# JuliaLinearAlgebra/ArnoldiMethod.jl

Measured on AMD Instinct MI355X. Metric: arnoldi_iters_per_sec, higher is better.
Workload: dtype f64

## Files before the change

### arnoldimethod.jl_amd/build.py

```python
from __future__ import annotations

import os
import shutil
import subprocess
from concurrent.futures import ThreadPoolExecutor

HERE = os.path.dirname(os.path.abspath(__file__))
CSRC = os.path.join(HERE, "csrc")
SRC = os.path.join(CSRC, "ks_hip.hip")
BLK = os.path.join(CSRC, "ks_block_inst.hip")
HEADERS = [os.path.join(CSRC, f) for f in ("ks_kernels.hpp", "ks_spmv_march.hpp", "ks_p2p.hpp", "ks_driver.hpp", "ks_smalldense.hpp", "ks_context.hpp", "ks_host_defs.hpp", "ks_csr_layout.hpp", "ks_halo_plan.hpp", "ks_halo.hpp", "ks_operators.hpp", "ks_sptrsv.hpp", "ks_tridiag_plan.hpp", "ks_tridiag.hpp", "ks_product.hpp", "ks_grid.hpp", "ks_grid_var.hpp", "ks_grid_box.hpp",
                                           "ks_workspace.hpp", "ks_backend.hpp", "ks_vectors.hpp", "ks_block.hpp", "ks_block_kernels.hpp", "ks_block_launch.hpp", "ks_block_mfma.hpp")]
DEPS = [SRC, BLK] + HEADERS + [os.path.join(HERE, "..", "include", "kschur.h")]
OUT = os.path.join(HERE, "libkschur_hip.so")
OBJDIR = os.path.join(HERE, "build")
BLK_DEPS = [BLK] + [os.path.join(CSRC, f) for f in ("ks_kernels.hpp", "ks_host_defs.hpp", "ks_p2p.hpp", "ks_block_kernels.hpp", "ks_block_launch.hpp", "ks_block_mfma.hpp")]
UNITS = {
    "ks_hip.o": (SRC, [], DEPS),
    "ks_block_inst0.o": (BLK, ["-DKS_BLK_PART=0"], BLK_DEPS),
    "ks_block_inst1.o": (BLK, ["-DKS_BLK_PART=1"], BLK_DEPS),
    "ks_block_inst2.o": (BLK, ["-DKS_BLK_PART=2"], BLK_DEPS),
}


def hipcc() -> str:
    for cand in (shutil.which("hipcc"), "/opt/rocm/bin/hipcc"):
        if cand and os.path.exists(cand):
            return cand
    raise RuntimeError("hipcc not found")


def needs_build() -> bool:
    if not os.path.exists(OUT):
        return True
    t = os.path.getmtime(OUT)
    return any(os.path.getmtime(d) > t for d in DEPS)


def _stale(obj: str, deps) -> bool:
    if not os.path.exists(obj):
        return True
    t = os.path.getmtime(obj)
    return any(os.path.getmtime(d) > t for d in deps)


def build(force: bool = False, verbose: bool = False) -> str:
    if not force and not needs_build():
        return OUT
    os.makedirs(OBJDIR, exist_ok=True)
    cc = hipcc()
    extra = os.environ.get("KS_EXTRA_HIPCC_FLAGS", "").split()
    jobs = []
    for name, (src, flags, deps) in UNITS.items():
        obj = os.path.join(OBJDIR, name)
        if force or extra or _stale(obj, deps):
            jobs.append([cc, "--offload-arch=gfx950", "-O3", "-std=c++17", "-fPIC", "-c", src, "-o", obj] + flags + extra)

    def run(cmd):
        if verbose:
            print(" ".join(cmd), flush=True)
        subprocess.check_call(cmd, cwd=CSRC)

    with ThreadPoolExecutor(max_workers=max(1, min(len(jobs), os.cpu_count() or 1))) as ex:
        list(ex.map(run, jobs))
    link = [cc, "--offload-arch=gfx950", "-shared", "-fPIC"] + [os.path.join(OBJDIR, n) for n in UNITS] + ["-o", OUT, "-L/opt/rocm/lib", "-lrccl", "-Wl,-rpath,/opt/rocm/lib"]
    run(link)
    return OUT


if __name__ == "__main__":
    print(build(force=True, verbose=True))
```

### arnoldimethod.jl_amd/csrc/ks_hip.hip

```cpp
#include <hip/hip_runtime.h>
#include <rccl/rccl.h>

#include <signal.h>
#include <unistd.h>

#include <algorithm>
#include <chrono>
#include <cmath>
#include <cstdio>
#include <cstdlib>
#include <cstring>
#include <memory>
#include <stdexcept>
#include <string>
#include <thread>
#include <unordered_map>
#include <vector>

#include "../../include/kschur.h"
#include "ks_driver.hpp"
#include "ks_kernels.hpp"
#include "ks_spmv_march.hpp"
#include "ks_block_kernels.hpp"
#include "ks_block_launch.hpp"

using ks::cplx;
using ksd::cd;
using ksd::DevState;
using ksd::kBlock;

#include "ks_context.hpp"
#include "ks_csr_layout.hpp"
#include "ks_halo_plan.hpp"
#include "ks_halo.hpp"
#include "ks_operators.hpp"
#include "ks_sptrsv.hpp"
#include "ks_tridiag.hpp"
#include "ks_product.hpp"
#include "ks_grid.hpp"
#include "ks_grid_var.hpp"
#include "ks_grid_box.hpp"
#include "ks_workspace.hpp"
#include "ks_block.hpp"
#include "ks_backend.hpp"
#include "ks_vectors.hpp"

namespace {

template <class F> int grid_operator_entry(ks_ctx* ctx, int dtype, ks_operator** out, const std::string& who, F make) {
  return guarded([&] {
    KS_REQUIRE(ctx && out, KS_ERR_ARGUMENT, "null argument");
    KS_REQUIRE(dtype == KS_F64 || dtype == KS_C64, KS_ERR_ARGUMENT, "unknown dtype");
    KS_REQUIRE(!ctx->distributed() && ctx->nranks == 1, KS_ERR_ARGUMENT, who + ": single-GPU contexts only (the grid is not partitioned across ranks)");
    ctx->use();
    *out = dtype == KS_F64 ? make(double{}, who) : make(cd{}, who);
  });
}

template <class F> int grid_host_entry(int dtype, const std::string& who, F fill) {
  return guarded([&] {
    KS_REQUIRE(dtype == KS_F64 || dtype == KS_C64, KS_ERR_ARGUMENT, "unknown dtype");
    if (dtype == KS_F64) fill(double{}, who);
    else fill(cplx{}, who);
  });
}

}

extern "C" {

const char* ks_last_error_string(void) { return g_last_error.c_str(); }

int ks_version(int* major, int* minor) {
  if (major) *major = KS_VERSION_MAJOR;
  if (minor) *minor = KS_VERSION_MINOR;
  return KS_OK;
}

int ks_ctx_create(int device, ks_ctx** out) {
  return guarded([&] {
    KS_REQUIRE(out, KS_ERR_ARGUMENT, "null out");
    auto c = std::make_unique<ks_ctx>();
    ctx_init_device(c.get(), device);
    *out = c.release();
  });
}

int ks_comm_unique_id(void* out128) {
  return guarded([&] {
    static_assert(sizeof(ncclUniqueId) == 128, "ncclUniqueId is 128 bytes");
    ncclUniqueId id;
    KS_NCCL(ncclGetUniqueId(&id));
    std::memcpy(out128, &id, 128);
  });
}

int ks_ctx_create_dist(int device, int rank, int nranks, const void* unique_id128, ks_ctx** out) {
  return guarded([&] {
    KS_REQUIRE(out && unique_id128, KS_ERR_ARGUMENT, "null argument");
    KS_REQUIRE(nranks >= 1 && rank >= 0 && rank < nranks, KS_ERR_ARGUMENT, "bad rank/nranks");
    auto c = std::make_unique<ks_ctx>();
    ctx_init_device(c.get(), device);
    c->rank = rank;
    c->nranks = nranks;
    ncclUniqueId id;
    std::memcpy(&id, unique_id128, 128);
    KS_NCCL(ncclCommInitRank(&c->comm, nranks, id, rank));
    const char* tr = std::getenv("KS_TRANSPORT");
    if (tr && std::string(tr) == "p2p") {
      p2p_alloc(c.get());
      hipIpcMemHandle_t mine;
      KS_HIP(hipIpcGetMemHandle(&mine, c->p2p.region));
      char* dbuf = nullptr;
      KS_HIP(hipMalloc(&dbuf, (size_t)64 * nranks));
      KS_HIP(hipMemcpy(dbuf + (size_t)64 * rank, &mine, 64, hipMemcpyHostToDevice));
      KS_NCCL(ncclAllGather(dbuf + (size_t)64 * rank, dbuf, 64, ncclChar, c->comm, c->stream));
      std::vector<char> all((size_t)64 * nranks);
      KS_HIP(hipMemcpyAsync(all.data(), dbuf, all.size(), hipMemcpyDeviceToHost, c->stream));
      KS_HIP(hipStreamSynchronize(c->stream));
      (void)hipFree(dbuf);
      p2p_attach(c.get(), all.data());
    }
    *out = c.release();
  });
}

int ks_ctx_create_hostcomm(int device, int rank, int nranks, ks_host_allreduce_fn allreduce, ks_host_exchange_fn exchange,
                           void* user, ks_ctx** out) {
  return guarded([&] {
    KS_REQUIRE(out && allreduce && exchange, KS_ERR_ARGUMENT, "null argument");
    KS_REQUIRE(nranks >= 1 && rank >= 0 && rank < nranks, KS_ERR_ARGUMENT, "bad rank/nranks");
    auto c = std::make_unique<ks_ctx>();
    ctx_init_device(c.get(), device);
    c->rank = rank;
    c->nranks = nranks;
    c->hc.allreduce = allreduce;
    c->hc.exchange = exchange;
    c->hc.user = user;
    *out = c.release();
  });
}

int ks_ctx_create_p2p(int device, int rank, int nranks, ks_ctx** out) {
  return guarded([&] {
    KS_REQUIRE(out, KS_ERR_ARGUMENT, "null out");
    KS_REQUIRE(nranks >= 1 && rank >= 0 && rank < nranks, KS_ERR_ARGUMENT, "bad rank/nranks");
    auto c = std::make_unique<ks_ctx>();
    ctx_init_device(c.get(), device);
    c->rank = rank;
    c->nranks = nranks;
    p2p_alloc(c.get());
    if (nranks == 1) p2p_attach(c.get(), nullptr);
    *out = c.release();
  });
}

int ks_ctx_p2p_handle(ks_ctx* ctx, void* out64) {
  return guarded([&] {
    KS_REQUIRE(ctx && out64, KS_ERR_ARGUMENT, "null argument");
    KS_REQUIRE(ctx->p2p.allocated, KS_ERR_ARGUMENT, "context was not created with ks_ctx_create_p2p");
    ctx->use();
    hipIpcMemHandle_t h;
    KS_HIP(hipIpcGetMemHandle(&h, ctx->p2p.region));
    std::memcpy(out64, &h, 64);
  });
}

int ks_ctx_p2p_attach(ks_ctx* ctx, const void* handles) {
  return guarded([&] {
    KS_REQUIRE(ctx && handles, KS_ERR_ARGUMENT, "null argument");
    ctx->use();
    p2p_attach(ctx, handles);
  });
}

int ks_ctx_destroy(ks_ctx* ctx) {
  return guarded([&] {
    if (!ctx) return;
    (void)hipSetDevice(ctx->device);
    if (ctx->stream) (void)hipStreamSynchronize(ctx->stream);
    if (ctx->comm) (void)ncclCommDestroy(ctx->comm);
    if (ctx->hc.stage) (void)hipHostFree(ctx->hc.stage);
    if (ctx->operr_h) (void)hipHostFree(ctx->operr_h);
    p2p_release(ctx);
    if (ctx->stream) (void)hipStreamDestroy(ctx->stream);
    delete ctx;
// ... 1579 lines not shown
```

### arnoldimethod.jl_amd/csrc/ks_operators.hpp

```cpp
#pragma once
struct ks_operator {
  ks_ctx* ctx = nullptr;
  int64_t n_local = 0, nnz = 0;
  int dtype = KS_F64;
  bool async_capable = true;
  double bytes_per_nnz = 0.0;
  double aux_bytes = 0.0;
  int layout = -1;
  double in_scale = 1.0;
  bool shift_store_cacheable = false;
  virtual ~ks_operator() = default;
  virtual void apply(const void* x, void* y, const DevState* st) = 0;
  virtual void apply_shifted(const void* x, void* y, double theta_re, double theta_im, double sigma, int64_t ld, const DevState* st);
};

namespace {

template <class D> struct CsrOp : ks_operator {
  void* rowptr = nullptr;
  bool ptr64 = false;
  int32_t* colidx = nullptr;
  D* val = nullptr;
  void* blkptr = nullptr;
  int32_t* blkrow = nullptr;
  int nblk = 0;
  std::vector<std::unique_ptr<CsrOp<D>>> cblocks;
  std::vector<char> cb_from_ghost;
  int cb_rpt = 0, cb_ni = 0;
  int ni = 7;
  bool row_gather = false;
  int nlong = 0;
  int32_t* blkpart = nullptr;
  D* lpart = nullptr;
  int32_t* lrow = nullptr;
  int32_t* lfirst = nullptr;
  int nstencil = 0;
  int stencil_mask_bytes = 1;
  void* smask = nullptr;
  void* smask2 = nullptr;
  ksd::StencilDict<D> sdict{};
  int nstencil_local = 0;
  mutable bool split_said = false;
  void* sliceptr = nullptr;
  int32_t* sperm = nullptr;
  int nslices = 0;
  int sell_un = 8;
  int64_t sell_entries = 0;
  int ndict = 0;
  int ndvi = 0;
  uint8_t* codes = nullptr;
  int32_t* ddelta = nullptr;
  int dvi_unroll = 8;
  int dvi_rpt = 1;
  Halo<D> halo;

  ~CsrOp() override {
    (void)hipFree(rowptr); (void)hipFree(colidx); (void)hipFree(val); (void)hipFree(blkptr); (void)hipFree(blkrow); (void)hipFree(smask); (void)hipFree(sliceptr); (void)hipFree(sperm); (void)hipFree(blkpart); (void)hipFree(lpart); (void)hipFree(lrow); (void)hipFree(lfirst);
    (void)hipFree(codes); (void)hipFree(ddelta);
  }
  void launch_csr_blocks(const D* x, D* y, const DevState* st, const D* yacc, int plain_store, ksd::ShiftArg<D> shift = ksd::ShiftArg<D>{}) {
    hipStream_t s = ctx->stream;
    auto go = [&](auto ip_tag) {
      using IP = decltype(ip_tag);
      auto launch = [&](auto ni_tag) {
        constexpr int NI = decltype(ni_tag)::value;
        if constexpr ((size_t)NI * kBlock * sizeof(D) <= (size_t)ksd::kSpmvCapBytes)
          ksd::k_spmv_csr<D, IP, false, NI><<<nblk, kBlock, 0, s>>>(static_cast<const IP*>(blkptr), blkrow, static_cast<const IP*>(rowptr), colidx, val, x,
                                                                    nullptr, y, n_local, nblk, st, nullptr, 0, 0, nullptr, nullptr, yacc, plain_store,
                                                                    ksd::HaloFused{}, ksd::HaloArgs{}, ksd::P2pDev{}, env_int("KS_SPMV_CSR_NT", 1) != 0, row_gather,
                                                                    plain_store ? ksd::ShiftArg<D>{} : shift);
        else
          throw KsError{KS_ERR_INTERNAL, "CSR row blocks of " + std::to_string(NI) + " x 256 entries exceed the LDS budget of this element type"};
      };
      switch (ni) {
        case 4: launch(std::integral_constant<int, 4>{}); break;
        case 7: launch(std::integral_constant<int, 7>{}); break;
        case 8: launch(std::integral_constant<int, 8>{}); break;
        case 12: launch(std::integral_constant<int, 12>{}); break;
        default: launch(std::integral_constant<int, 16>{}); break;
      }
    };
    if (ptr64) go(int64_t{});
    else go(int32_t{});
  }
  bool shift_on = false;
  D shift_theta{};
  double shift_sigma = 1.0;
  bool shift_plain() const {
    static const int env = env_int("KS_SHIFT_PLAIN", -1);
    return env >= 0 ? env != 0 : shift_store_cacheable;
  }
  static bool march_on() {
    return env_int("KS_STENCIL_MARCH", 1) != 0;
  }
  int march_slots(int ntiles) const {
    const int env = env_int("KS_MARCH_S", 0);
    int S = 192;
    if (env > 0) S = env;
    else {
      int64_t P = 0;
      for (int k = 0; k < nstencil; ++k) P = std::max<int64_t>(P, std::llabs((long long)sdict.delta[k]));
      const int64_t per = P / 512 + 1;
      if (per >= 16 && per <= 224) S = (int)(per * ((160 + per - 1) / per)) <= 224 ? (int)(per * ((160 + per - 1) / per)) : (int)per;
    }
    S = std::min(S, std::max(1, (ntiles + 7) / 8));
    return S;
  }
  void launch_march(const D* x, D* y, int nt, const DevState* st, hipStream_t s) const {
    if constexpr (std::is_same<D, double>::value) {
      const int sh = shift_on ? (1 | (shift_plain() ? 2 : 0)) : 0;
      const uint16_t* m2 = static_cast<const uint16_t*>(smask2);
      const int G = 8 * march_slots(nt);
      int kown = -1;
      for (int k = 0; k < nstencil; ++k)
        if (sdict.delta[k] == 0) kown = k;
      auto go = [&](auto ns_tag, auto ko_tag) {
        ksd::k_spmv_stencil_march<decltype(ns_tag)::value, decltype(ko_tag)::value><<<G, kBlock, 0, s>>>(m2, sdict, x, y, n_local, nt, st, sh, shift_theta, shift_sigma);
      };
      const int window = env_int("KS_MARCH_WINDOW", 1);
      if (window && nstencil == 7 && kown == 3) {
        bool shape = std::llabs((long long)sdict.delta[0]) > 256 && std::llabs((long long)sdict.delta[6]) > 256;
        unsigned odd = 0;
        for (int k = 1; k <= 5; ++k) {
          shape = shape && std::llabs((long long)sdict.delta[k]) <= 256;
          if (sdict.delta[k] & 1) odd |= 1u << k;
        }
        const int zmarch = env_int("KS_MARCH_Z", 1), zr_env = env_int("KS_MARCH_ZR", 0);
        const int64_t Pz = sdict.delta[6];
        if (shape && zmarch && sdict.delta[0] == -Pz && (Pz & 1) == 0 && Pz >= 8 * 8 * 512) {
          const int nzp = (int)((n_local + Pz - 1) / Pz), cmax = (int)(((Pz + 511) / 512 + 7) / 8);
          int nzr = zr_env > 0 ? zr_env : std::max(1, (288 + cmax / 2) / cmax);
          nzr = std::max(1, std::min(nzr, nzp / 4));
          if (nzp >= 8) {
            auto gz = [&](auto odd_tag) {
              ksd::k_spmv_stencil_marchz<7, 0x3eu, decltype(odd_tag)::value, 3, 0, 6><<<8 * cmax * nzr, kBlock, 0, s>>>(m2, sdict, x, y, n_local, nzr, st, sh, shift_theta, shift_sigma);
            };
            if (odd == 0x14u) gz(std::integral_constant<unsigned, 0x14u>{});
            else if (odd == 0x36u) gz(std::integral_constant<unsigned, 0x36u>{});
            else gz(std::integral_constant<unsigned, 0x3eu>{});
            return;
          }
        }
        if (shape) {
          auto gw = [&](auto odd_tag) {
            ksd::k_spmv_stencil_marchw<7, 0x3eu, decltype(odd_tag)::value, 3><<<G, kBlock, 0, s>>>(m2, sdict, x, y, n_local, nt, st, sh, shift_theta, shift_sigma);
          };
          if (odd == 0x14u) gw(std::integral_constant<unsigned, 0x14u>{});
          else if (odd == 0x36u) gw(std::integral_constant<unsigned, 0x36u>{});
          else gw(std::integral_constant<unsigned, 0x3eu>{});
          return;
        }
      }
      using M1 = std::integral_constant<int, -1>;
      if (nstencil == 7 && kown == 3) go(std::integral_constant<int, 7>{}, std::integral_constant<int, 3>{});
      else if (nstencil == 5 && kown == 2) go(std::integral_constant<int, 5>{}, std::integral_constant<int, 2>{});
      else if (nstencil == 3 && kown == 1) go(std::integral_constant<int, 3>{}, std::integral_constant<int, 1>{});
      else switch (nstencil) {
        case 1: go(std::integral_constant<int, 1>{}, M1{}); break;
        case 2: go(std::integral_constant<int, 2>{}, M1{}); break;
        case 3: go(std::integral_constant<int, 3>{}, M1{}); break;
        case 4: go(std::integral_constant<int, 4>{}, M1{}); break;
        case 5: go(std::integral_constant<int, 5>{}, M1{}); break;
        case 6: go(std::integral_constant<int, 6>{}, M1{}); break;
        case 7: go(std::integral_constant<int, 7>{}, M1{}); break;
        default: go(std::integral_constant<int, 8>{}, M1{}); break;
      }
    }
  }
  ksd::ShiftArg<D> shift_arg() const {
    ksd::ShiftArg<D> a;
    a.on = shift_on ? 1 : 0;
    a.theta = shift_theta;
    a.sigma = shift_sigma;
    return a;
  }
  void apply_shifted(const void* xv, void* yv, double tre, double tim, double sigma, int64_t ld, const DevState* st) override {
    const int fuse = env_int("KS_SHIFT_FUSED", 1);
    const bool fused = fuse && n_local > 0 && nlong == 0;
    if (!fused) { ks_operator::apply_shifted(xv, yv, tre, tim, sigma, ld, st); return; }
    shift_on = true;
    if constexpr (sizeof(D) == 8) shift_theta = tre; else shift_theta = D{tre, tim};
    shift_sigma = sigma;
    try { apply(xv, yv, st); } catch (...) { shift_on = false; throw; }
    shift_on = false;
  }
  void apply(const void* xv, void* yv, const DevState* st) override {
    const D* x = static_cast<const D*>(xv);
    D* y = static_cast<D*>(yv);
    hipStream_t s = ctx->stream;
    const typename Halo<D>::Begun begun = halo.begin(x, st, n_local > 0 && cblocks.empty() && ndvi == 0 && nslices == 0);
    const ksd::HaloFused& hf = begun.hf;
    const D* xg = begun.xg;
    if (n_local > 0 && !cblocks.empty()) {
      ProfScope ps(ctx, KSP_SPMV, (double)nnz * bytes_per_nnz + aux_bytes + 2.0 * sizeof(D) * n_local);
      if (cb_rpt) {
        ksd::CbArgs<D> a{};
        a.nb = (int)cblocks.size();
        for (int b = 0; b < a.nb; ++b) {
          a.rowptr[b] = static_cast<const int32_t*>(cblocks[b]->rowptr);
          a.colidx[b] = cblocks[b]->colidx;
          a.val[b] = cblocks[b]->val;
          a.xb[b] = (!cb_from_ghost.empty() && cb_from_ghost[b]) ? xg : nullptr;
        }
        const int nt = (int)((n_local + (int64_t)kBlock * cb_rpt - 1) / ((int64_t)kBlock * cb_rpt));
        auto go = [&](auto ni_tag, auto rpt_tag) {
          constexpr int NI = decltype(ni_tag)::value, RPT = decltype(rpt_tag)::value;
          if constexpr ((size_t)NI * kBlock * sizeof(D) <= (size_t)ksd::kSpmvCapBytes)
            ksd::k_spmv_csr_cb<D, NI, RPT><<<nt, kBlock, 0, s>>>(a, x, y, n_local, nt, st, shift_arg());
          else
            throw KsError{KS_ERR_INTERNAL, "column-blocked CSR: LDS depth exceeds the budget of this element type"};
        };
        auto by_rpt = [&](auto ni_tag) {
          switch (cb_rpt) {
            case 1: go(ni_tag, std::integral_constant<int, 1>{}); break;
            case 2: go(ni_tag, std::integral_constant<int, 2>{}); break;
            case 4: go(ni_tag, std::integral_constant<int, 4>{}); break;
            case 8: go(ni_tag, std::integral_constant<int, 8>{}); break;
            default: go(ni_tag, std::integral_constant<int, 16>{}); break;
          }
        };
        if (cb_ni == 8) by_rpt(std::integral_constant<int, 8>{});
        else by_rpt(std::integral_constant<int, 16>{});
        KS_HIP(hipGetLastError());
        return;
      }
      for (size_t b = 0; b < cblocks.size(); ++b) cblocks[b]->launch_csr_blocks(x, y, st, b > 0 ? y : nullptr, b + 1 < cblocks.size() ? 1 : 0, shift_arg());
      KS_HIP(hipGetLastError());
      return;
    }
    if (n_local > 0) {
      ProfScope ps(ctx, KSP_SPMV, (double)nnz * bytes_per_nnz + aux_bytes + 2.0 * sizeof(D) * n_local);
      const uint32_t* hseq = nullptr;
      auto with_ip = [&](auto f) {
        if (ptr64) f(int64_t{});
        else f(int32_t{});
      };
      if (nstencil > 0 && halo.plan.nghost == 0 && smask2 && n_local >= 2 && env_int("KS_STENCIL_PAIRS", 1)) {
        const int nt = (int)(((n_local + 1) / 2 + kBlock - 1) / kBlock);
        if constexpr (std::is_same<D, double>::value) {
          if (stencil_mask_bytes == 1 && nstencil <= 8 && march_on()) {
            launch_march(x, y, nt, st, s);
            KS_HIP(hipGetLastError());
            return;
          }
        }
        if (stencil_mask_bytes == 1)
          ksd::k_spmv_stencil2<D, uint16_t><<<nt, kBlock, 0, s>>>(static_cast<const uint16_t*>(smask2), sdict, nstencil, x, y, n_local, nt, st, shift_on ? (1 | (shift_plain() ? 2 : 0)) : 0, shift_theta, shift_sigma);
        else
          ksd::k_spmv_stencil2<D, uint64_t><<<nt, kBlock, 0, s>>>(static_cast<const uint64_t*>(smask2), sdict, nstencil, x, y, n_local, nt, st, shift_on ? (1 | (shift_plain() ? 2 : 0)) : 0, shift_theta, shift_sigma);
        KS_HIP(hipGetLastError());
        return;
      }
      if (nstencil > 0 && halo.plan.nghost > 0 && !halo.p2p && smask2 && (stencil_mask_bytes == 1 || stencil_mask_bytes == 4) && n_local >= 2 * kBlock) {
        if constexpr (std::is_same<D, double>::value) {
          static const int split_env = env_int("KS_DIST_SPLIT", 1);
          const int nt1 = (int)((n_local + kBlock - 1) / kBlock);
          const int nlow = (int)((halo.plan.ghost_lo_end + kBlock - 1) / kBlock), first_high = (int)(halo.plan.ghost_hi_begin / kBlock);
          const int nhigh = nt1 - first_high;
          if (split_env && env_int("KS_STENCIL_PAIRS", 1) && nlow <= first_high && 4 * (nlow + nhigh) <= nt1 && nlow + nhigh > 0) {
            const int nt2 = (int)(((n_local + 1) / 2 + kBlock - 1) / kBlock);
            static const int split_dbg = env_int("KS_DIST_SPLIT_DEBUG", 0);
            if (split_dbg && !split_said) {
              split_said = true;
              std::fprintf(stderr, "[split] rows %lld: paired kernel on all of them (%d of %d slots), ghost-aware kernel on %d + %d boundary tiles of %d\n", (long long)n_local, nstencil_local, nstencil, nlow, nhigh, nt1);
            }
            const int shf = shift_on ? (1 | (shift_plain() ? 2 : 0)) : 0;
            ksd::HaloFused h0{};
            const int nsl = nstencil_local >= 1 ? nstencil_local : nstencil;
            if (stencil_mask_bytes == 1) {
              ksd::k_spmv_stencil2<D, uint16_t><<<nt2, kBlock, 0, s>>>(static_cast<const uint16_t*>(smask2), sdict, nsl, x, y, n_local, nt2, st, shf, shift_theta, shift_sigma);
              ksd::k_spmv_stencil<D, uint8_t, 1><<<nlow + nhigh, kBlock, 0, s>>>(static_cast<const uint8_t*>(smask), sdict, nstencil, x, xg, y, n_local,
                                                                                std::max<int64_t>(halo.plan.nghost, 0), nlow + nhigh, st, h0, halo.hargs, ctx->p2p.dev, shift_on ? 1 : 0,
                                                                                shift_theta, shift_sigma, nlow, first_high - nlow);
            } else {
              ksd::k_spmv_stencil2<D, uint64_t><<<nt2, kBlock, 0, s>>>(static_cast<const uint64_t*>(smask2), sdict, nsl, x, y, n_local, nt2, st, shf, shift_theta, shift_sigma);
              ksd::k_spmv_stencil<D, uint32_t, 1><<<nlow + nhigh, kBlock, 0, s>>>(static_cast<const uint32_t*>(smask), sdict, nstencil, x, xg, y, n_local,
                                                                                 std::max<int64_t>(halo.plan.nghost, 0), nlow + nhigh, st, h0, halo.hargs, ctx->p2p.dev, shift_on ? 1 : 0,
                                                                                 shift_theta, shift_sigma, nlow, first_high - nlow);
            }
            KS_HIP(hipGetLastError());
            return;
          }
// ... 118 lines not shown
    KS_HIP(hipGetLastError());
  }
};

struct HostCallbackOp : ks_operator {
  ks_host_apply_fn fn = nullptr;
  void* user = nullptr;
  void* xh = nullptr;
  void* yh = nullptr;
  ~HostCallbackOp() override { (void)hipHostFree(xh); (void)hipHostFree(yh); }
  void apply(const void* x, void* y, const DevState*) override {
    const size_t bytes = (size_t)n_local * (dtype == KS_F64 ? 8 : 16);
    KS_HIP(hipMemcpyAsync(xh, x, bytes, hipMemcpyDeviceToHost, ctx->stream));
    KS_HIP(hipStreamSynchronize(ctx->stream));
    const int64_t nd = n_local * (dtype == KS_F64 ? 1 : 2);
    if (in_scale != 1.0) {
      double* xd = static_cast<double*>(xh);
      for (int64_t i = 0; i < nd; ++i) xd[i] *= in_scale;
    }
    const int rc = fn(user, xh, yh);
    KS_REQUIRE(rc == 0, KS_ERR_OPERATOR, "host operator callback returned " + std::to_string(rc));
    if (in_scale != 1.0) {
      const double back = 1.0 / in_scale;
      double* yd = static_cast<double*>(yh);
      for (int64_t i = 0; i < nd; ++i) yd[i] *= back;
    }
    KS_HIP(hipMemcpyAsync(y, yh, bytes, hipMemcpyHostToDevice, ctx->stream));
  }
};

struct DeviceCallbackOp : ks_operator {
  ks_device_apply_fn fn = nullptr;
  void* user = nullptr;
  void apply(const void* x, void* y, const DevState*) override {
    const int rc = fn(user, x, y, (void*)ctx->stream);
    KS_REQUIRE(rc == 0, KS_ERR_OPERATOR, "device operator callback returned " + std::to_string(rc));
  }
};

template <class I> inline int64_t idx_at(const void* p, int64_t i) { return (int64_t) static_cast<const I*>(p)[i]; }

template <class D>
void build_csr_host(int64_t nrows, int64_t ncols, int64_t nnz, const void* ptr, const void* idx, const void* val,
                    int layout, int base, int itype, std::vector<int64_t>& rp, std::vector<int32_t>& ci,
                    std::vector<D>& vv) {
  auto P = [&](int64_t i) { return (itype == KS_I32 ? idx_at<int32_t>(ptr, i) : idx_at<int64_t>(ptr, i)) - base; };
  auto J = [&](int64_t i) { return (itype == KS_I32 ? idx_at<int32_t>(idx, i) : idx_at<int64_t>(idx, i)) - base; };
  const D* v = static_cast<const D*>(val);
  KS_REQUIRE(nrows < (int64_t)2147483647 && ncols < (int64_t)2147483647, KS_ERR_ARGUMENT, "matrix order must fit int32");
  {
    const int64_t np = (layout == KS_CSR ? nrows : ncols);
    int64_t prev = P(0);
    KS_REQUIRE(prev == 0, KS_ERR_ARGUMENT, layout == KS_CSR ? "row pointer does not match nnz" : "column pointer does not match nnz");
    for (int64_t i = 1; i <= np; ++i) {
      const int64_t cur = P(i);
      KS_REQUIRE(cur >= prev && cur <= nnz, KS_ERR_ARGUMENT, "pointer array is not monotone within [0, nnz]");
      prev = cur;
    }
    KS_REQUIRE(prev == nnz, KS_ERR_ARGUMENT, layout == KS_CSR ? "row pointer does not match nnz" : "column pointer does not match nnz");
  }
  rp.assign(nrows + 1, 0);
  ci.resize(nnz);
  vv.resize(nnz);
  if (layout == KS_CSR) {
    for (int64_t i = 0; i <= nrows; ++i) rp[i] = P(i);
    for (int64_t p = 0; p < nnz; ++p) {
      const int64_t c = J(p);
      KS_REQUIRE(c >= 0 && c < ncols, KS_ERR_ARGUMENT, "column index out of range");
      ci[p] = (int32_t)c;
      vv[p] = v[p];
    }
  } else {
    for (int64_t p = 0; p < nnz; ++p) {
      const int64_t r = J(p);
      KS_REQUIRE(r >= 0 && r < nrows, KS_ERR_ARGUMENT, "row index out of range");
      rp[r + 1]++;
    }
    for (int64_t i = 0; i < nrows; ++i) rp[i + 1] += rp[i];
    std::vector<int64_t> fill(rp.begin(), rp.end() - 1);
    for (int64_t c = 0; c < ncols; ++c)
      for (int64_t p = P(c); p < P(c + 1); ++p) {
        const int64_t r = J(p);
        const int64_t q = fill[r]++;
        ci[q] = (int32_t)c;
        vv[q] = v[p];
      }
  }
}

inline void build_csr_dist_host(int64_t nrows, int64_t nghost, int64_t nnz, const int64_t* rowptr, const int32_t* colidx,
                                std::vector<int64_t>& rp, std::vector<int32_t>& ci) {
  KS_REQUIRE(nrows < (int64_t)2147483647 && nghost < (int64_t)2147483647 - nrows, KS_ERR_ARGUMENT, "local-extended column range must fit int32");
  rp.resize(nrows + 1);
  KS_REQUIRE(rowptr[0] == 0 && rowptr[nrows] == nnz, KS_ERR_ARGUMENT, "row pointer does not match nnz");
  for (int64_t i = 0; i <= nrows; ++i) {
    KS_REQUIRE(i == 0 || (rowptr[i] >= rowptr[i - 1] && rowptr[i] <= nnz), KS_ERR_ARGUMENT, "pointer array is not monotone within [0, nnz]");
    rp[i] = rowptr[i];
  }
  ci.assign(colidx, colidx + nnz);
  for (int64_t p = 0; p < nnz; ++p)
    KS_REQUIRE(ci[p] >= 0 && ci[p] < nrows + nghost, KS_ERR_ARGUMENT, "local-extended column index out of range");
}

inline void* upload_ptr(const std::vector<int64_t>& v, bool ptr64) {
  void* d = nullptr;
  const size_t cnt = v.size();
  if (ptr64) {
    KS_HIP(hipMalloc(&d, std::max<size_t>(cnt * 8, 16)));
    KS_HIP(hipMemcpy(d, v.data(), cnt * 8, hipMemcpyHostToDevice));
  } else {
    std::vector<int32_t> t(v.begin(), v.end());
    KS_HIP(hipMalloc(&d, std::max<size_t>(cnt * 4, 16)));
    KS_HIP(hipMemcpy(d, t.data(), cnt * 4, hipMemcpyHostToDevice));
  }
  return d;
}

template <class T> T* upload_vec(const T* v, size_t cnt, size_t pad, bool zero = false) {
  void* d = nullptr;
  KS_HIP(hipMalloc(&d, (cnt + pad) * sizeof(T)));
  if (zero) KS_HIP(hipMemset(d, 0, (cnt + pad) * sizeof(T)));
  if (cnt) KS_HIP(hipMemcpy(d, v, cnt * sizeof(T), hipMemcpyHostToDevice));
  return static_cast<T*>(d);
}
template <class T> T* upload_vec(const std::vector<T>& v, size_t pad, bool zero = false) { return upload_vec(v.data(), v.size(), pad, zero); }

template <class D>
CsrOp<D>* upload(ks_ctx* ctx, const CsrPlan<D>& P, int64_t nrows, int64_t nnz, const std::vector<int64_t>& rp, const std::vector<int32_t>& ci,
                 const std::vector<D>& vv) {
  auto op = std::make_unique<CsrOp<D>>();
  op->ctx = ctx;
  op->n_local = nrows;
  op->nnz = nnz;
  op->dtype = sizeof(D) == 8 ? KS_F64 : KS_C64;
  op->layout = P.layout;
  op->ptr64 = P.ptr64;
  op->bytes_per_nnz = P.bytes_per_nnz;
  op->aux_bytes = P.aux_bytes;
  op->ndict = P.ndict;
  constexpr size_t kPad16 = 16 / sizeof(D);
  switch (P.layout) {
    case KS_LAYOUT_STENCIL: {
      op->nstencil = P.nstencil;
      op->nstencil_local = P.nstencil_local;
      op->stencil_mask_bytes = P.stencil_mask_bytes;
      for (int k = 0; k < ksd::kStencilSlots; ++k) {
        op->sdict.delta[k] = k < P.nstencil ? P.sdelta[k] : 0;
        op->sdict.val[k] = k < P.nstencil ? P.sval[k] : D{};
      }
      const size_t pad = (size_t)(round_up(nrows + 2, 8) - nrows);
      if (P.stencil_mask_bytes == 1) op->smask = upload_vec(P.mask8, pad, true);
      else op->smask = upload_vec(P.mask32, pad, true);
      op->smask2 = op->smask;
      break;
    }
    case KS_LAYOUT_DVI:
      op->ndvi = P.ndvi;
      op->dvi_unroll = P.dvi_unroll;
      op->dvi_rpt = P.dvi_rpt;
      op->rowptr = upload_ptr(rp, P.ptr64);
      op->codes = upload_vec(P.codes, 64, true);
      op->ddelta = upload_vec(P.ddelta, 256 - P.ddelta.size());
      op->val = upload_vec(P.dval, 256 - P.dval.size());
      break;
    case KS_LAYOUT_SELL:
    case KS_LAYOUT_SELL_VI:
      op->nslices = P.nslices;
      op->sell_un = P.sell_un;
      op->sell_entries = P.sell_entries;
      op->sliceptr = upload_ptr(P.sliceptr, P.ptr64);
      op->colidx = upload_vec(P.sell_col, 4);
      if (P.ndict > 0) op->val = upload_vec(P.dict, 256 - P.dict.size());
      else op->val = upload_vec(P.sell_val, kPad16);
      if (!P.sell_perm.empty()) op->sperm = upload_vec(P.sell_perm, 0);
      break;
    case KS_LAYOUT_CSR_CB:
      for (const CsrPlan<D>& cb : P.cblocks)
        op->cblocks.emplace_back(upload<D>(ctx, cb, nrows, (int64_t)cb.sub_ci.size(), cb.sub_rp, cb.sub_ci, cb.sub_vv));
      op->cb_from_ghost = P.cb_from_ghost;
      op->cb_rpt = P.cb_rpt;
      op->cb_ni = P.cb_ni;
      break;
    default: {
      op->ni = P.ni;
      op->row_gather = P.row_gather;
      op->nlong = P.nlong;
      op->nblk = P.nblk;
      op->blkptr = upload_ptr(P.blkptr, P.ptr64);
      op->blkrow = upload_vec(P.blkrow, P.blkrow.size() < 4 ? 4 - P.blkrow.size() : 0);
      if (P.nlong > 0) {
        op->blkpart = upload_vec(P.blkpart, 0);
        KS_HIP(hipMalloc(&op->lpart, (size_t)P.lfirst.back() * sizeof(D)));
        op->lrow = upload_vec(P.lrow, 0);
        op->lfirst = upload_vec(P.lfirst, 0);
      }
      op->rowptr = upload_ptr(rp, P.ptr64);
      if (P.ndict > 0) {
        op->colidx = upload_vec(P.packed, 2 + 4);
        op->val = upload_vec(P.dict, 256 - P.dict.size());
      } else {
        op->colidx = upload_vec(ci.data(), (size_t)nnz, 2 + 4);
        op->val = upload_vec(vv.data(), (size_t)nnz, 2 + kPad16);
      }
    }
  }
  return op.release();
}

template <class D>
CsrOp<D>* make_csr(ks_ctx* ctx, int64_t nrows, int64_t nnz, const std::vector<int64_t>& rp, const std::vector<int32_t>& ci,
                   const std::vector<D>& vv, CbMode cb_mode = CbMode::None, int64_t nghost = 0, int64_t nlow = 0) {
  const CsrPlan<D> plan = plan_csr<D>(CsrHost<D>{nrows, nnz, rp, ci, vv}, FormatRequest::from_env(), cb_mode, nghost, nlow, ctx->num_cu);
  return upload<D>(ctx, plan, nrows, nnz, rp, ci, vv);
}

}

inline void ks_operator::apply_shifted(const void* x, void* y, double theta_re, double theta_im, double sigma, int64_t ld, const DevState* st) {
  apply(x, y, st);
  ProfScope ps(ctx, KSP_SCALE, 3.0 * (double)n_local * (dtype == KS_F64 ? 8.0 : 16.0));
  const int nbk = (int)std::max<int64_t>(1, std::min<int64_t>((int64_t)ctx->num_cu * 8, ld / (2 * kBlock) + 1));
  if (dtype == KS_F64) {
    ksd::k_shift_scale<double><<<nbk, kBlock, 0, ctx->stream>>>(static_cast<double*>(y), static_cast<const double*>(x), theta_re, sigma, ld, st);
  } else {
    ksd::k_shift_scale<cd><<<nbk, kBlock, 0, ctx->stream>>>(static_cast<cd*>(y), static_cast<const cd*>(x), cd{theta_re, theta_im}, sigma, ld, st);
  }
  KS_HIP(hipGetLastError());
}
```

### arnoldimethod.jl_amd/csrc/ks_spmv_march.hpp

```cpp
#pragma once

#include <algorithm>
#include <type_traits>

#include "ks_kernels.hpp"

namespace ksd {

typedef double f64x2m __attribute__((ext_vector_type(2)));

__device__ __forceinline__ double and_mask(double p, int bm) {
  const uint64_t u = __builtin_bit_cast(uint64_t, p);
  const uint32_t lo = (uint32_t)u & (uint32_t)bm, hi = (uint32_t)(u >> 32) & (uint32_t)bm;
  return __builtin_bit_cast(double, ((uint64_t)hi << 32) | lo);
}

__device__ __forceinline__ int march_tile(int xcd, int slot, int it, int S, int ntiles, int& tend) {
  const int q = ntiles >> 3, r = ntiles & 7;
  const int t0 = xcd < r ? xcd * (q + 1) : r * (q + 1) + (xcd - r) * q;
  tend = t0 + (xcd < r ? q + 1 : q);
  return t0 + slot + it * S;
}

__device__ __forceinline__ void march_ld16(f64x2m& dst, uint32_t voff, const void* sbase) {
// ... 385 lines not shown
  const bool plain_st = (shifted & 2) != 0;
  const bool lane_in = off0 + 2 * (int64_t)threadIdx.x + 1 < P;
  const int nst = (off0 + 128 * (int64_t)wave + 1 < P) ? 1 : 0;
  auto r0_of = [&](int z) { return (int64_t)z * P + off0; };
  auto win_ok = [&](int z) { const int64_t r0 = r0_of(z); return z >= 0 && r0 - 256 >= 0 && r0 + kTile + 256 <= n; };
  auto interior = [&](int z) { return win_ok(z) && r0_of(z) + kTile <= n && (win_ok(z + 1) || r0_of(z + 1) >= n); };

  auto edge = [&](int z) {
    const int64_t r = r0_of(z) + 2 * (int64_t)threadIdx.x;
    if (!lane_in || r >= n) return;
    const bool two = r + 1 < n;
    const uint32_t m = mask2[r >> 1];
    const uint32_t m0 = m & 0xffu, m1 = m >> 8;
    const int64_t cmax = n - 2;
    double s0 = 0.0, s1 = 0.0;
#pragma unroll
    for (int k = 0; k < NSLOT; ++k) {
      const int64_t c = r + d.delta[k];
      int64_t lo = c < 0 ? 0 : (c > cmax ? cmax : c);
      if (cmax < 0) lo = 0;
      const int sh = (int)(c - lo);
      double xa, xb;
      if (n >= 2) ld_pair_u(x + lo, xa, xb);
      else { xa = x[0]; xb = x[0]; }
      const double v0 = sh == 1 ? xb : xa, v1 = sh == -1 ? xa : xb;
      const double p0 = mul_nc(d.val[k], v0), p1 = mul_nc(d.val[k], v1);
      s0 = ((m0 >> k) & 1u) ? add_(s0, p0) : s0;
      s1 = ((m1 >> k) & 1u) ? add_(s1, p1) : s1;
    }
    if (shifted) {
      double x0, x1;
      if (two) ld_pair_u(x + r, x0, x1);
      else { x0 = x[r]; x1 = x0; }
      s0 = scl(sub_s(s0, mul_(theta, x0)), sigma);
      s1 = scl(sub_s(s1, mul_(theta, x1)), sigma);
    }
    if (two) {
      if (plain_st) st_pack(y + r, make_double2(s0, s1));
      else st_pack_nt(y + r, make_double2(s0, s1));
    } else {
      if (plain_st) y[r] = s0;
      else st_elem_nt(y + r, s0);
    }
  };
  int zi0 = za, zi1 = zb;
  while (zi0 < zi1 && !interior(zi0)) ++zi0;
  while (zi1 > zi0 && !interior(zi1 - 1)) --zi1;
  if (zi0 > za || zi1 < zb) {
    for (int z = za; z < zb; ++z)
      if (z < zi0 || z >= zi1) edge(z);
    asm volatile("s_waitcnt vmcnt(0)" ::: "memory");
  }
  if (zi0 >= zi1) return;

  auto issue_w = [&](int zz, int zsafe, int buf) {
    const int zu = win_ok(zz) ? zz : zsafe;
    const double* bw = x + (r0_of(zu) - 256 + (int64_t)wave * 128);
    uint32_t ldst = win0 + (uint32_t)buf * (uint32_t)kWinB + (uint32_t)wave * 1024u;
    asm volatile("" : "+s"(bw));
    asm volatile("" : "+s"(ldst));
    asm volatile("s_nop 4" ::: "memory");
    march_glds16(lane_w, bw, ldst);
    if (wave + kWaves < kPieces) march_glds16(lane_w + (uint32_t)kWaves * 1024u, bw, ldst + (uint32_t)kWaves * 1024u);
  };
  auto issue_m = [&](int zz, uint32_t& m) {
    const uint16_t* bm = mask2 + (r0_of(zz) >> 1);
    asm volatile("" : "+s"(bm));
    asm volatile("s_nop 4" ::: "memory");
    march_ld_u16(m, lane_m, bm);
  };
  f64x2m prev;
  {
    const double* bp = x + (zi0 >= 1 ? r0_of(zi0 - 1) : r0_of(zi0));
    asm volatile("" : "+s"(bp));
    asm volatile("s_nop 4" ::: "memory");
    march_ld16(prev, lane_b, bp);
  }
  uint32_t mA, mB;
  issue_w(zi0, zi0, 0);
  issue_w(zi0 + 1, zi0, 1);
  if constexpr (NB == 4) issue_w(zi0 + 2, zi0, 2);
  issue_m(zi0, mA);
  int bc = 0;
  auto step = [&](int z, uint32_t& m, uint32_t& mnext, bool first, bool has_next) {
    constexpr int NW_LATE = NB == 4 ? 2 : 0;
    if (first) asm volatile("s_waitcnt vmcnt(0)\n\ts_barrier" ::: "memory");
    else if (nst == 0) asm volatile("s_waitcnt vmcnt(%0)\n\ts_barrier" :: "n"(NW_LATE) : "memory");
    else asm volatile("s_waitcnt vmcnt(%0)\n\ts_barrier" :: "n"(NW_LATE + 1) : "memory");
    asm volatile("" : "+v"(m));
    if (first) asm volatile("" : "+v"(prev));
    const int bn = bc + 1 == NB ? 0 : bc + 1, b2 = bc == 0 ? NB - 1 : bc - 1;
    if constexpr (NB == 3) {
      issue_w(z + 2, z, b2);
      if (has_next) issue_m(z + 1, mnext);
    } else {
      if (has_next) issue_m(z + 1, mnext);
      issue_w(z + 3, z, b2);
    }
    const unsigned char* w = &win[0][0] + bc * kWinB + (256 * 8) + threadIdx.x * 16;
    f64x2m v[NSLOT];
#pragma unroll
    for (int k = 0; k < NSLOT; ++k) {
      if ((NEARM >> k) & 1u) {
        const int off = (int)d.delta[k] * 8;
        if (((ODDM >> k) & 1u) == 0) {
          v[k] = *reinterpret_cast<const f64x2m*>(w + off);
        } else {
          typedef double f64x2u8 __attribute__((ext_vector_type(2), aligned(8)));
          const f64x2u8 p = *reinterpret_cast<const f64x2u8*>(w + off);
          v[k].x = p.x;
          v[k].y = p.y;
        }
      }
    }
    v[KFM] = prev;
    v[KFP] = *reinterpret_cast<const f64x2m*>(&win[0][0] + bn * kWinB + (256 * 8) + threadIdx.x * 16);
    const int m0 = (int)(m & 0xffu), m1 = (int)(m >> 8);
    double s0 = 0.0, s1 = 0.0;
#pragma unroll
    for (int k = 0; k < NSLOT; ++k) {
      const double p0 = mul_nc(d.val[k], v[k].x), p1 = mul_nc(d.val[k], v[k].y);
      s0 = add_(s0, and_mask(p0, __builtin_amdgcn_sbfe(m0, k, 1)));
      s1 = add_(s1, and_mask(p1, __builtin_amdgcn_sbfe(m1, k, 1)));
    }
    if (shifted) {
      s0 = scl(sub_s(s0, mul_(theta, v[KOWN].x)), sigma);
      s1 = scl(sub_s(s1, mul_(theta, v[KOWN].y)), sigma);
    }
    prev = v[KOWN];
    f64x2m o2;
    o2.x = s0;
    o2.y = s1;
    double* by = y + r0_of(z);
    asm volatile("" : "+s"(by));
    if (lane_in) march_st16(lane_b, o2, by, plain_st);
    bc = bn;
  };
  int z = zi0;
  bool first = true;
  for (;;) {
    const bool h1 = z + 1 < zi1;
    step(z, mA, mB, first, h1);
    first = false;
    if (!h1) break;
    ++z;
    const bool h2 = z + 1 < zi1;
    step(z, mB, mA, false, h2);
    if (!h2) break;
    ++z;
  }
  asm volatile("s_waitcnt vmcnt(0)" ::: "memory");
}

}
```

Measured before the change: 4813.

## Add box-geometry z-march stencil SpMV that computes masks instead of loading them

At setup the code checks whether the 7-point stencil mask matches a plain 3D box. If it does, it dispatches a new z-marching kernel with 1024-row tiles and 512 threads. That kernel derives the boundary masks arithmetically from x/y/z coordinates instead of reading the mask array, and triple-buffers the x windows in LDS with explicit vmcnt waits. The aim is to remove mask-load traffic and improve load overlap in the memory-bound SpMV. The costs are extra host validation at setup and a risk of wrong vmcnt counting or broken coverage at edges.

```diff
diff --git a/arnoldimethod.jl_amd/build.py b/arnoldimethod.jl_amd/build.py
--- a/arnoldimethod.jl_amd/build.py
+++ b/arnoldimethod.jl_amd/build.py
@@ -9,7 +9,7 @@
 CSRC = os.path.join(HERE, "csrc")
 SRC = os.path.join(CSRC, "ks_hip.hip")
 BLK = os.path.join(CSRC, "ks_block_inst.hip")
-HEADERS = [os.path.join(CSRC, f) for f in ("ks_kernels.hpp", "ks_spmv_march.hpp", "ks_p2p.hpp", "ks_driver.hpp", "ks_smalldense.hpp", "ks_context.hpp", "ks_host_defs.hpp", "ks_csr_layout.hpp", "ks_halo_plan.hpp", "ks_halo.hpp", "ks_operators.hpp", "ks_sptrsv.hpp", "ks_tridiag_plan.hpp", "ks_tridiag.hpp", "ks_product.hpp", "ks_grid.hpp", "ks_grid_var.hpp", "ks_grid_box.hpp",
+HEADERS = [os.path.join(CSRC, f) for f in ("ks_kernels.hpp", "ks_spmv_march.hpp", "ks_p2p.hpp", "ks_driver.hpp", "ks_smalldense.hpp", "ks_context.hpp", "ks_host_defs.hpp", "ks_csr_layout.hpp", "ks_halo_plan.hpp", "ks_stencil_geom.hpp", "ks_halo.hpp", "ks_operators.hpp", "ks_sptrsv.hpp", "ks_tridiag_plan.hpp", "ks_tridiag.hpp", "ks_product.hpp", "ks_grid.hpp", "ks_grid_var.hpp", "ks_grid_box.hpp",
                                            "ks_workspace.hpp", "ks_backend.hpp", "ks_vectors.hpp", "ks_block.hpp", "ks_block_kernels.hpp", "ks_block_launch.hpp", "ks_block_mfma.hpp")]
 DEPS = [SRC, BLK] + HEADERS + [os.path.join(HERE, "..", "include", "kschur.h")]
 OUT = os.path.join(HERE, "libkschur_hip.so")
diff --git a/arnoldimethod.jl_amd/csrc/ks_hip.hip b/arnoldimethod.jl_amd/csrc/ks_hip.hip
--- a/arnoldimethod.jl_amd/csrc/ks_hip.hip
+++ b/arnoldimethod.jl_amd/csrc/ks_hip.hip
@@ -32,6 +32,7 @@
 #include "ks_context.hpp"
 #include "ks_csr_layout.hpp"
 #include "ks_halo_plan.hpp"
+#include "ks_stencil_geom.hpp"
 #include "ks_halo.hpp"
 #include "ks_operators.hpp"
 #include "ks_sptrsv.hpp"
diff --git a/arnoldimethod.jl_amd/csrc/ks_operators.hpp b/arnoldimethod.jl_amd/csrc/ks_operators.hpp
--- a/arnoldimethod.jl_amd/csrc/ks_operators.hpp
+++ b/arnoldimethod.jl_amd/csrc/ks_operators.hpp
@@ -40,6 +40,7 @@
   void* smask2 = nullptr;
   ksd::StencilDict<D> sdict{};
   int nstencil_local = 0;
+  StencilGeom geom;
   mutable bool split_said = false;
   void* sliceptr = nullptr;
   int32_t* sperm = nullptr;
@@ -128,6 +129,18 @@
         const int zmarch = env_int("KS_MARCH_Z", 1), zr_env = env_int("KS_MARCH_ZR", 0);
         const int64_t Pz = sdict.delta[6];
         if (shape && zmarch && sdict.delta[0] == -Pz && (Pz & 1) == 0 && Pz >= 8 * 8 * 512) {
+          if (geom.box && n_local / Pz >= 8 && env_int("KS_MARCH_GEOM", 1) != 0) {
+            constexpr int kTileG = 1024, kThreadsG = 512, kSlotsG = 2 * 32 * 4;
+            const int nzp = (int)(n_local / Pz), cmax = (int)(((Pz + kTileG - 1) / kTileG + 7) / 8);
+            int nzr = zr_env > 0 ? zr_env : std::max(1, (kSlotsG + cmax / 2) / cmax);
+            nzr = std::max(1, std::min(nzr, nzp / 4));
+            auto gg = [&](auto odd_tag) {
+              ksd::k_spmv_stencil_marchg<decltype(odd_tag)::value, kTileG, kThreadsG><<<8 * cmax * nzr, kThreadsG, 0, s>>>(m2, sdict, x, y, n_local, nzr, st, sh, shift_theta, shift_sigma);
+            };
+            if (odd == 0x14u) gg(std::integral_constant<unsigned, 0x14u>{});
+            else gg(std::integral_constant<unsigned, 0x36u>{});
+            return;
+          }
           const int nzp = (int)((n_local + Pz - 1) / Pz), cmax = (int)(((Pz + 511) / 512 + 7) / 8);
           int nzr = zr_env > 0 ? zr_env : std::max(1, (288 + cmax / 2) / cmax);
           nzr = std::max(1, std::min(nzr, nzp / 4));
@@ -552,6 +565,8 @@
       if (P.stencil_mask_bytes == 1) op->smask = upload_vec(P.mask8, pad, true);
       else op->smask = upload_vec(P.mask32, pad, true);
       op->smask2 = op->smask;
+      if (std::is_same<D, double>::value && P.stencil_mask_bytes == 1 && P.nstencil == P.nstencil_local)
+        op->geom = stencil_geometry(P.sdelta.data(), P.nstencil, nrows, P.mask8.data(), P.mask8.size());
       break;
     }
     case KS_LAYOUT_DVI:
diff --git a/arnoldimethod.jl_amd/csrc/ks_spmv_march.hpp b/arnoldimethod.jl_amd/csrc/ks_spmv_march.hpp
--- a/arnoldimethod.jl_amd/csrc/ks_spmv_march.hpp
+++ b/arnoldimethod.jl_amd/csrc/ks_spmv_march.hpp
@@ -561,4 +561,214 @@
   asm volatile("s_waitcnt vmcnt(0)" ::: "memory");
 }
 
-}
+__device__ __forceinline__ void march_wait_vm(int c) {
+  switch (c) {
+    case 0: asm volatile("s_waitcnt vmcnt(0)" ::: "memory"); break;
+    case 1: asm volatile("s_waitcnt vmcnt(1)" ::: "memory"); break;
+    case 2: asm volatile("s_waitcnt vmcnt(2)" ::: "memory"); break;
+    case 3: asm volatile("s_waitcnt vmcnt(3)" ::: "memory"); break;
+    case 4: asm volatile("s_waitcnt vmcnt(4)" ::: "memory"); break;
+    case 5: asm volatile("s_waitcnt vmcnt(5)" ::: "memory"); break;
+    case 6: asm volatile("s_waitcnt vmcnt(6)" ::: "memory"); break;
+    default: asm volatile("s_waitcnt vmcnt(7)" ::: "memory"); break;
+  }
+}
+
+template <unsigned ODDM, int TILE, int TW>
+__global__ void __launch_bounds__(TW)
+    k_spmv_stencil_marchg(const uint16_t* __restrict__ mask2, const StencilDict<double> d, const double* __restrict__ x,
+                          double* __restrict__ y, int64_t n, int nzr, const DevState* __restrict__ st, int shifted, double theta,
+                          double sigma) {
+  constexpr int NSLOT = 7, KOWN = 3, KFM = 0, KFP = 6;
+  constexpr unsigned NEARM = 0x3eu;
+  constexpr int PPL = TILE / (2 * TW), kWinB = (TILE + 512) * 8, kPieces = (TILE + 512) / 128, kWaves = TW / 64;
+  constexpr int kRounds = (kPieces + kWaves - 1) / kWaves;
+  static_assert(TW == 256 || TW == 512, "four or eight waves");
+  static_assert((PPL == 1 || PPL == 2) && PPL * 2 * TW == TILE, "one or two pairs per lane");
+  static_assert(3 * kWinB <= 60 * 1024, "three window buffers in at most 60 KiB");
+  static_assert(kRounds + 2 * PPL <= 7, "march_wait_vm counts up to 7");
+  if (st && st->breakdown >= 0) return;
+  __shared__ __attribute__((aligned(16))) unsigned char win[3][kWinB];
+  const int64_t P = d.delta[KFP];
+  const int nx = d.delta[5], ny = (int)(P / nx);
+  const int nz = (int)(n / P), ntp = (int)((P + TILE - 1) / TILE);
+  const int xcd = blockIdx.x & 7, slot = blockIdx.x >> 3;
+  int cnt;
+  const int tj0 = march_tile(xcd, 0, 0, 0, ntp, cnt);
+  cnt -= tj0;
+  if (cnt <= 0) return;
+  const int zr = slot / cnt, tile = tj0 + slot % cnt;
+  if (zr >= nzr) return;
+  const int za = (int)((int64_t)zr * nz / nzr), zb = (int)((int64_t)(zr + 1) * nz / nzr);
+  const int64_t off0 = (int64_t)tile * TILE;
+  const int wave = __builtin_amdgcn_readfirstlane(threadIdx.x >> 6);
+  const uint32_t lane_w = (threadIdx.x & 63u) * 16u;
+  const uint32_t win0 = (uint32_t)(uintptr_t)&win[0][0];
+  const bool plain_st = (shifted & 2) != 0;
+  const int nw = (kPieces - wave + kWaves - 1) / kWaves;
+  uint32_t lane_b[PPL];
+  bool lane_in[PPL];
+  bool wave_has[PPL];
+  int mA[PPL], mB[PPL];
+  int nst = 0;
+#pragma unroll
+  for (int j = 0; j < PPL; ++j) {
+    const int64_t o = off0 + (int64_t)j * 2 * TW + 2 * (int64_t)threadIdx.x;
+    lane_b[j] = (uint32_t)(j * 2 * TW + 2 * (int)threadIdx.x) * 8u;
+    lane_in[j] = o + 1 < P;
+    wave_has[j] = off0 + (int64_t)j * 2 * TW + 128 * (int64_t)wave + 1 < P;
+    nst += wave_has[j] ? 1 : 0;
+    const int oa = (int)o, ob = oa + 1;
+    const int ya = oa / nx, xa = oa - ya * nx, yb = ob / nx, xb = ob - yb * nx;
+    mA[j] = 0x08 | (ya > 0 ? 0x02 : 0) | (xa > 0 ? 0x04 : 0) | (xa < nx - 1 ? 0x10 : 0) | (ya < ny - 1 ? 0x20 : 0);
+    mB[j] = 0x08 | (yb > 0 ? 0x02 : 0) | (xb > 0 ? 0x04 : 0) | (xb < nx - 1 ? 0x10 : 0) | (yb < ny - 1 ? 0x20 : 0);
+  }
+  auto r0_of = [&](int z) { return (int64_t)z * P + off0; };
+  auto interior = [&](int z) { const int64_t r0 = r0_of(z); return z >= 0 && z < nz && r0 - 256 >= 0 && r0 + TILE + 256 <= n; };
+
+  auto edge = [&](int z) {
+#pragma unroll
+    for (int j = 0; j < PPL; ++j) {
+      const int64_t r = r0_of(z) + (int64_t)j * 2 * TW + 2 * (int64_t)threadIdx.x;
+      if (!lane_in[j] || r >= n) continue;
+      const bool two = r + 1 < n;
+      const uint32_t m = mask2[r >> 1];
+      const uint32_t m0 = m & 0xffu, m1 = m >> 8;
+      const int64_t cmax = n - 2;
+      double s0 = 0.0, s1 = 0.0;
+#pragma unroll
+      for (int k = 0; k < NSLOT; ++k) {
+        const int64_t c = r + d.delta[k];
+        int64_t lo = c < 0 ? 0 : (c > cmax ? cmax : c);
+        if (cmax < 0) lo = 0;
+        const int sh = (int)(c - lo);
+        double xa, xb;
+        if (n >= 2) ld_pair_u(x + lo, xa, xb);
+        else { xa = x[0]; xb = x[0]; }
+        const double v0 = sh == 1 ? xb : xa, v1 = sh == -1 ? xa : xb;
+        const double p0 = mul_nc(d.val[k], v0), p1 = mul_nc(d.val[k], v1);
+        s0 = ((m0 >> k) & 1u) ? add_(s0, p0) : s0;
+        s1 = ((m1 >> k) & 1u) ? add_(s1, p1) : s1;
+      }
+      if (shifted) {
+        double x0, x1;
+        if (two) ld_pair_u(x + r, x0, x1);
+        else { x0 = x[r]; x1 = x0; }
+        s0 = scl(sub_s(s0, mul_(theta, x0)), sigma);
+        s1 = scl(sub_s(s1, mul_(theta, x1)), sigma);
+      }
+      if (two) {
+        if (plain_st) st_pack(y + r, make_double2(s0, s1));
+        else st_pack_nt(y + r, make_double2(s0, s1));
+      } else {
+        if (plain_st) y[r] = s0;
+        else st_elem_nt(y + r, s0);
+      }
+    }
+  };
+  int zi0 = za, zi1 = zb;
+  while (zi0 < zi1 && !interior(zi0)) ++zi0;
+  while (zi1 > zi0 && !interior(zi1 - 1)) --zi1;
+  if (zi0 > za || zi1 < zb) {
+    for (int z = za; z < zb; ++z)
+      if (z < zi0 || z >= zi1) edge(z);
+    asm volatile("s_waitcnt vmcnt(0)" ::: "memory");
+  }
+  if (zi0 >= zi1) return;
+
+  auto issue_w = [&](int zz, int buf) {
+    const double* bw = x + (r0_of(zz) - 256 + (int64_t)wave * 128);
+    uint32_t ldst = win0 + (uint32_t)buf * (uint32_t)kWinB + (uint32_t)wave * 1024u;
+    asm volatile("" : "+s"(bw));
+    asm volatile("" : "+s"(ldst));
+    asm volatile("s_nop 4" ::: "memory");
+#pragma unroll
+    for (int i = 0; i < kRounds; ++i)
+      if (wave + i * kWaves < kPieces) march_glds16(lane_w + (uint32_t)(i * kWaves) * 1024u, bw, ldst + (uint32_t)(i * kWaves) * 1024u);
+  };
+  f64x2m prev[PPL];
+  f64x2m top[PPL];
+  f64x2m acc[PPL];
+  {
+    const int zt = zi1 < nz ? zi1 : zi1 - 1;
+    const double* bp = x + (zi0 >= 1 ? r0_of(zi0 - 1) : r0_of(zi0));
+    const double* bt = x + r0_of(zt);
+    asm volatile("" : "+s"(bp));
+    asm volatile("" : "+s"(bt));
+    asm volatile("s_nop 4" ::: "memory");
+#pragma unroll
+    for (int j = 0; j < PPL; ++j) march_ld16(prev[j], lane_b[j], bp);
+#pragma unroll
+    for (int j = 0; j < PPL; ++j) march_ld16(top[j], lane_in[j] ? lane_b[j] : 0u, bt);
+  }
+  issue_w(zi0, 0);
+  if (zi0 + 1 < zi1) issue_w(zi0 + 1, 1);
+  auto finish = [&](int zrow, int j, f64x2m nxt, int fpm) {
+    double s0 = add_(acc[j].x, and_mask(mul_nc(d.val[KFP], nxt.x), fpm));
+    double s1 = add_(acc[j].y, and_mask(mul_nc(d.val[KFP], nxt.y), fpm));
+    if (shifted) {
+      s0 = scl(sub_s(s0, mul_(theta, prev[j].x)), sigma);
+      s1 = scl(sub_s(s1, mul_(theta, prev[j].y)), sigma);
+    }
+    f64x2m o2;
+    o2.x = s0;
+    o2.y = s1;
+    double* by = y + r0_of(zrow);
+    asm volatile("" : "+s"(by));
+    if (wave_has[j]) {
+      if (lane_in[j]) march_st16(lane_b[j], o2, by, plain_st);
+    }
+  };
+  int bc = 0;
+  int i = 0;
+  for (int z = zi0; z < zi1; ++z, ++i) {
+    march_wait_vm((z + 1 < zi1 ? nw : 0) + nst * ((i >= 3 ? 1 : 0) + (i >= 2 ? 1 : 0)));
+    asm volatile("s_waitcnt lgkmcnt(0)\n\ts_barrier" ::: "memory");
+    if (i == 0) {
+#pragma unroll
+      for (int j = 0; j < PPL; ++j) {
+        asm volatile("" : "+v"(prev[j]));
+        asm volatile("" : "+v"(top[j]));
+      }
+    }
+    if (z + 2 < zi1) issue_w(z + 2, bc == 0 ? 2 : bc - 1);
+    const int fm = z > 0 ? -1 : 0;
+#pragma unroll
+    for (int j = 0; j < PPL; ++j) {
+      const unsigned char* w = &win[0][0] + bc * kWinB + (256 * 8) + lane_b[j];
+      f64x2m v[NSLOT];
+#pragma unroll
+      for (int k = 0; k < NSLOT; ++k) {
+        if ((NEARM >> k) & 1u) {
+          const int off = (int)d.delta[k] * 8;
+          if (((ODDM >> k) & 1u) == 0) {
+            v[k] = *reinterpret_cast<const f64x2m*>(w + off);
+          } else {
+            typedef double f64x2u8 __attribute__((ext_vector_type(2), aligned(8)));
+            const f64x2u8 p = *reinterpret_cast<const f64x2u8*>(w + off);
+            v[k].x = p.x;
+            v[k].y = p.y;
+          }
+        }
+      }
+      v[KFM] = prev[j];
+      if (i > 0) finish(z - 1, j, v[KOWN], -1);
+      double s0 = 0.0, s1 = 0.0;
+#pragma unroll
+      for (int k = 0; k < KFP; ++k) {
+        const double p0 = mul_nc(d.val[k], v[k].x), p1 = mul_nc(d.val[k], v[k].y);
+        s0 = add_(s0, and_mask(p0, k == KFM ? fm : __builtin_amdgcn_sbfe(mA[j], k, 1)));
+        s1 = add_(s1, and_mask(p1, k == KFM ? fm : __builtin_amdgcn_sbfe(mB[j], k, 1)));
+      }
+      acc[j].x = s0;
+      acc[j].y = s1;
+      prev[j] = v[KOWN];
+    }
+    bc = bc == 2 ? 0 : bc + 1;
+  }
+#pragma unroll
+  for (int j = 0; j < PPL; ++j) finish(zi1 - 1, j, top[j], zi1 < nz ? -1 : 0);
+  asm volatile("s_waitcnt vmcnt(0)" ::: "memory");
+}
+
+}
diff --git a/arnoldimethod.jl_amd/csrc/ks_stencil_geom.hpp b/arnoldimethod.jl_amd/csrc/ks_stencil_geom.hpp
--- /dev/null
+++ b/arnoldimethod.jl_amd/csrc/ks_stencil_geom.hpp
@@ -0,0 +1,33 @@
+#pragma once
+
+#include <cstddef>
+#include <cstdint>
+
+struct StencilGeom {
+  bool box = false;
+  int64_t nx = 0, ny = 0, nz = 0;
+};
+
+inline uint8_t stencil_box_mask(int64_t x, int64_t y, int64_t z, int64_t nx, int64_t ny, int64_t nz) {
+  return (uint8_t)((z > 0 ? 0x01u : 0u) | (y > 0 ? 0x02u : 0u) | (x > 0 ? 0x04u : 0u) | 0x08u | (x < nx - 1 ? 0x10u : 0u) |
+                   (y < ny - 1 ? 0x20u : 0u) | (z < nz - 1 ? 0x40u : 0u));
+}
+
+inline StencilGeom stencil_geometry(const int32_t* delta, int nslot, int64_t n, const uint8_t* mask8, size_t nmask) {
+  StencilGeom g;
+  if (nslot != 7 || n <= 0 || !delta || !mask8 || nmask != (size_t)n) return g;
+  const int64_t nx = delta[5], P = delta[6];
+  if (nx < 2 || P <= nx || P % nx != 0 || n % P != 0) return g;
+  if (delta[0] != -P || delta[1] != -nx || delta[2] != -1 || delta[3] != 0 || delta[4] != 1) return g;
+  const int64_t ny = P / nx, nz = n / P;
+  int64_t r = 0;
+  for (int64_t z = 0; z < nz; ++z)
+    for (int64_t y = 0; y < ny; ++y)
+      for (int64_t x = 0; x < nx; ++x, ++r)
+        if (mask8[r] != stencil_box_mask(x, y, z, nx, ny, nz)) return g;
+  g.box = true;
+  g.nx = nx;
+  g.ny = ny;
+  g.nz = nz;
+  return g;
+}
```

Result: faster. 4949, median of 6 (+2.8%).
